# MrTornado24/IDE-3D

Measured on AMD Instinct MI355X. Metric: 512x512 RGB+seg frames/s @96 depth samples (whole job), higher is better.
Workload: dtype f32 (3x3 convs + MLPs: fp32 operands as 3 bf16 pieces, 6 products, f32 accumulate); 1 GPU; BASELINE config 2: random-init ide3d-ffhq-64-512, G.mapping + G.synthesis (64 render -> 512, 96 samples, RGB + 19-class seg) + uint8 frames, batch 4 seeds per GPU; global_batch=4, parallelism=dp1, conv_arithmetic=bf16x6, conv_arithmetic_is_library_default=True

## Files before the change

ide-3d_amd/csrc/modconv.hip:

```cpp
#include "common.h"
#include "knobs.h"
#include <stdlib.h>
#include <string.h>
#include <type_traits>

namespace ide3d {

typedef float f32x16 __attribute__((ext_vector_type(16)));

#ifdef IDE3D_MC_TRACE
__device__ unsigned long long g_mc_dbg[256];
#define IDE3D_MC_TS(k) { const unsigned long long now_ = __builtin_readcyclecounter(); mc_acc[k] += now_ - mc_last; mc_last = now_; }
#else
#define IDE3D_MC_TS(k)
#endif

enum { MODE_CONV3 = 0, MODE_CONV1 = 1, MODE_TCONV3 = 2, MODE_TCONV3A = 3, MODE_CONV3S2 = 4 };

template <int MODE> struct ModeCfg;
template <> struct ModeCfg<MODE_CONV3>  { static constexpr int KC = 4, WTAPS = 9, MAXT = 9; };
template <> struct ModeCfg<MODE_CONV1>  { static constexpr int KC = 16, WTAPS = 1, MAXT = 1; };
template <> struct ModeCfg<MODE_CONV3S2> { static constexpr int KC = 4, WTAPS = 9, MAXT = 9; };
template <> struct ModeCfg<MODE_TCONV3> { static constexpr int KC = 4, WTAPS = 9, MAXT = 4; };
template <> struct ModeCfg<MODE_TCONV3A> { static constexpr int KC = 4, WTAPS = 9, MAXT = 9; };

template <int MODE, int BIG, int TI, int PH, int PW>
struct McCfg {
    static constexpr int NWV = 4, NT = 64 * NWV;
    static constexpr int BN = TI * PH * PW;
    static_assert(BN == 64 || BN == 128 || BN == 256, "pixel tile must hold 64, 128 or 256 pixels");
    static constexpr int NCLS = (MODE == MODE_TCONV3A) ? 4 : 1;
    using MC = ModeCfg<MODE>;
    static constexpr int KC = MC::KC, WTAPS = MC::WTAPS, MAXT = MC::MAXT;
    static constexpr int WM = BIG ? 2 : 1, WN = NWV / WM;
    static constexpr int MTW = (BIG == 1) ? 2 : 1;
    static constexpr int NTW = (BN / 32) / WN;
    static constexpr int BM = WM * MTW * 32;
    static constexpr int STRIDE = (MODE == MODE_CONV3S2) ? 2 : 1;
    static constexpr int HALO = (MODE == MODE_CONV1 || MODE == MODE_CONV3S2) ? 0 : 1;
    static constexpr int HP = (MODE == MODE_CONV3S2) ? 2 * PH + 1 : PH + 2 * HALO;
    static constexpr int HW = (MODE == MODE_CONV3S2) ? 2 * PW + 1 : PW + 2 * HALO;
    static constexpr int XW = (MODE == MODE_CONV1) ? PW : (MODE == MODE_CONV3S2) ? ((HW + 3) & ~3) : ((PW == 16) ? 48 : HW + 2);
    static constexpr int XS = HP * XW;
    static constexpr int XI = KC * XS;
    static constexpr int LDS_W = MAXT * KC * BM;
    static constexpr int LDS_X = TI * XI;
    static constexpr int NW4 = (LDS_W / 4 + NT - 1) / NT;
    static constexpr int VW = (MODE == MODE_CONV1 && PH == 1 && PW % 4 == 0) ? 4 : 1;
    static constexpr int NXE = (TI * KC * HP * HW / VW + NT - 1) / NT;
};

template <int N>
__device__ __forceinline__ int sel(const int (&a)[N], int t) {
    int v = a[0];
#pragma unroll
    for (int i = 1; i < N; ++i) v = (t == i) ? a[i] : v;
    return v;
}

__host__ __device__ inline int mc_bm(int cout) { return cout > 96 ? 128 : (cout > 32 ? 64 : 32); }
__host__ __device__ inline int mc_kc(int k) { return k == 3 ? 4 : 16; }

__global__ void __launch_bounds__(256)
modconv_pack_kernel(const float* __restrict__ w, int64_t w_batch_stride, int nbatch, int cout, int cin, int taps, int bm, int kc,
                    int mblocks, int cchunks, float* __restrict__ out) {
    const int64_t total = (int64_t)nbatch * mblocks * cchunks * taps * kc * bm;
    const int64_t stride = (int64_t)gridDim.x * blockDim.x;
    for (int64_t i = (int64_t)blockIdx.x * blockDim.x + threadIdx.x; i < total; i += stride) {
        int64_t r = i;
        const int co_l = (int)(r % bm); r /= bm;
        const int cil = (int)(r % kc); r /= kc;
        const int tap = (int)(r % taps); r /= taps;
        const int cc = (int)(r % cchunks); r /= cchunks;
        const int mb = (int)(r % mblocks); r /= mblocks;
        const int nb = (int)r;
        const int co = mb * bm + co_l, ci = cc * kc + cil;
        out[i] = (co < cout && ci < cin) ? w[nb * w_batch_stride + ((int64_t)co * cin + ci) * taps + tap] : 0.f;
    }
}

struct ConvGeom {
    int tiles_x[4], tiles_y[4];
    int tile_base[5];
    int img_groups;
    int mblocks, cchunks, split_k, chunks_per_split;
    int oh, ow;
};

template <int OFF_BYTES>
__device__ __forceinline__ float lds_read_async(unsigned addr) {
    float v;
    asm volatile("ds_read_b32 %0, %1 offset:%2" : "=v"(v) : "v"(addr), "n"(OFF_BYTES));
    return v;
}
template <int PENDING>
__device__ __forceinline__ void lds_wait(float& first) { asm volatile("s_waitcnt lgkmcnt(%1)" : "+v"(first) : "n"(PENDING)); }
__device__ __forceinline__ void lds_pin(float& v) { asm volatile("" : "+v"(v)); }
__device__ __forceinline__ unsigned lds_addr(const float* p) { return (unsigned)(size_t)p; }

template <class F, int... Is>
__device__ __forceinline__ void static_for_impl(F&& f, std::integer_sequence<int, Is...>) { (f(std::integral_constant<int, Is>{}), ...); }
template <int N, class F>
__device__ __forceinline__ void static_for(F&& f) { static_for_impl(f, std::make_integer_sequence<int, N>{}); }

template <int MODE, int XW>
__host__ __device__ constexpr int tap_patch_offset(int t) {
    return (MODE == MODE_CONV1) ? 0
         : (MODE == MODE_TCONV3A) ? ((t / 3 == 2) ? 0 : 1) * XW + ((t % 3 == 2) ? 0 : 1)
         : (t / 3) * XW + (t % 3);
}
template <int MODE>
__host__ __device__ constexpr int tap_class(int t) { return (MODE == MODE_TCONV3A) ? ((t / 3) & 1) * 2 + ((t % 3) & 1) : 0; }

__device__ __forceinline__ void amax_acc(float& m, float v) { m = fmaxf(m, fabsf(v)); }
__device__ __forceinline__ void amax_commit(float* y_amax, int n, float v, bool) {
    if (v > 0.f) amax_raise(y_amax, n, v);
}

template <int MODE, int TI, int PH, int PW, int NWV, int NCLS, int MTW, int NTW, int BM, int SCRATCH, int ROWPAR = -1>
__device__ __forceinline__ void modconv_finish(const ide3d_modconv_params& p, float* __restrict__ partial, const ConvGeom& g,
                                               f32x16 (&acc)[NCLS][MTW][NTW], float* s_w, int mb, int n0, int y0, int x0, int split, int cls,
                                               int wm, int wn, int lp, const float* __restrict__ row_unscale = nullptr, float x_unscale = 1.f,
                                               int team_tid = -1, float* amax_scratch = nullptr) {
    constexpr int NT = 64 * NWV;
    const int tid = team_tid >= 0 ? team_tid : (int)threadIdx.x, lane = tid & 63, wid = tid >> 6, half = lane >> 5;
    const int cpy = cls >> 1, cpx = cls & 1;
    const bool raw = (g.split_k > 1);
    float* const s_dm = s_w;
    float* const s_bi = s_w + TI * BM;
    for (int e = tid; e < TI * BM; e += NT) {
        const int rl = e % BM, co = mb * BM + rl, n = min(n0 + e / BM, p.n - 1);
        float d = (!raw && p.dcoefs && co < p.cout) ? p.dcoefs[(int64_t)n * p.cout + co] : 1.f;
        if (row_unscale) d *= row_unscale[co] * x_unscale;
        s_dm[e] = d;
        if (e < BM) s_bi[e] = (!raw && p.bias && co < p.cout) ? p.bias[co] : 0.f;
    }
    __syncthreads();
    float* const dst = raw ? partial + (int64_t)split * p.n * p.cout * g.oh * g.ow : p.y;
    const int64_t pitch = (!raw && p.y_pitch > 0) ? p.y_pitch : g.ow;
    const float e_alpha = (!raw && p.act == 3) ? p.alpha : 1.f, e_gain = raw ? 1.f : p.gain;
    const float e_clamp = (!raw && p.clamp >= 0.f) ? p.clamp : __builtin_inff();
    const float e_nstr = (!raw && p.noise) ? p.noise_strength : 0.f;
    auto finish = [&](float v, float d, float nz, float bb) {
        v *= d; v += nz; v += bb;
        v = (v > 0.f) ? v : v * e_alpha;
        v *= e_gain;
        return fminf(fmaxf(v, -e_clamp), e_clamp);
    };
    const bool want_amax = !raw && p.y_amax != nullptr;
    float amax_tile = 0.f;
    constexpr int QX = (MODE == MODE_TCONV3A) ? 2 : 1, QY = NCLS / QX;
    static_assert(ROWPAR < 0 || (MODE == MODE_TCONV3A && NCLS == 2), "one row parity = two column classes");
    constexpr int TW = 32 * QX, TP = TW + 8;
    constexpr int AVAIL = SCRATCH - (TI + 1) * BM;
    constexpr int RR = (MODE == MODE_TCONV3 || PW % 4 != 0) ? 0 : (AVAIL >= NWV * 32 * TP) ? 32 : (AVAIL >= NWV * 16 * TP) ? 16 : (AVAIL >= NWV * 8 * TP) ? 8 : 0;
    if constexpr (RR > 0) {
        typedef float f32x4u __attribute__((ext_vector_type(4), aligned(4)));
        float* const T = s_w + (TI + 1) * BM + wid * (RR * TP);
#pragma unroll
        for (int qy = 0; qy < QY; ++qy)
#pragma unroll
// ... 958 lines not shown
        const char* src = uniform_ptr(xbase + (int64_t)t * 128);
#pragma unroll
        for (int c = 0; c < NCH; ++c)
#pragma unroll
            for (int e = 0; e < 8; ++e) {
                xr[B][c][e] = *reinterpret_cast<const float*>(src + (c * 16 + e) * plane + x_lane);
            }
    };
    typedef float f32x4a __attribute__((ext_vector_type(4)));
    const float* const bi = s_bi + 4 * half;
    f32x16 acc[MT];
    auto compute = [&](auto buf_tag) {
        constexpr int B = decltype(buf_tag)::value;
#pragma unroll
        for (int m = 0; m < MT; ++m)
#pragma unroll
            for (int g = 0; g < 4; ++g) {
                const f32x4a b4 = *reinterpret_cast<const f32x4a*>(bi + m * 32 + 8 * g);
#pragma unroll
                for (int k = 0; k < 4; ++k) acc[m][4 * g + k] = b4[k];
            }
#pragma unroll
        for (int c = 0; c < NCH; ++c) {
            u32x4 bfrag[PARTS];
            {
                unsigned pk[4][PARTS];
#pragma unroll
                for (int e = 0; e < 4; ++e) split_pair<PARTS>(xr[B][c][2 * e], xr[B][c][2 * e + 1], pk[e]);
#pragma unroll
                for (int q = 0; q < PARTS; ++q) bfrag[q] = u32x4{pk[0][q], pk[1][q], pk[2][q], pk[3][q]};
            }
            const u32x4* sa = s_a + c * K::A_UNITS + half * K::ROWS + l32;
            constexpr int MG = (MT % 2 == 0) ? 2 : 1;
#pragma unroll
            for (int m0 = 0; m0 < MT; m0 += MG) {
                u32x4 af[MG][PARTS];
#pragma unroll
                for (int g = 0; g < MG; ++g)
#pragma unroll
                    for (int q = 0; q < PARTS; ++q) af[g][q] = sa[q * 2 * K::ROWS + (m0 + g) * 32];
                constexpr int NQA = PARTS;
#pragma unroll
                for (int qa = 0; qa < NQA; ++qa)
#pragma unroll
                    for (int qb = 0; qa + qb < NQA; ++qb)
#pragma unroll
                        for (int g = 0; g < MG; ++g)
                            acc[m0 + g] = __builtin_amdgcn_mfma_f32_32x32x16_bf16(__builtin_bit_cast(bf16x8, af[g][qa]), __builtin_bit_cast(bf16x8, bfrag[qb]), acc[m0 + g], 0, 0, 0);
            }
        }
    };
    const bool all_rows = (p.cout == K::ROWS), unit_gain = (e_gain == 1.f), want_amax = (p.y_amax != nullptr);
    auto finish = [&](int t) {
        char* dst = uniform_ptr(ybase + (int64_t)t * 128);
        auto rows = [&](auto all_tag, auto gain_tag) {
            constexpr bool ALL = decltype(all_tag)::value, UNIT = decltype(gain_tag)::value;
#pragma unroll
            for (int m = 0; m < MT; ++m)
#pragma unroll
                for (int r = 0; r < 16; ++r) {
                    const int row_u = m * 32 + 8 * (r >> 2) + (r & 3);
                    if (ALL || row_u + 4 * half < p.cout) {
                        float v = acc[m][r];
                        if (!UNIT) v *= e_gain;
                        v = __builtin_amdgcn_fmed3f(v, -e_clamp, e_clamp);
                        *reinterpret_cast<float*>(dst + row_u * plane + y_lane) = v;
                        if (want_amax) amax_acc(amax, v);
                    }
                }
        };
        if (all_rows) { if (unit_gain) rows(std::true_type{}, std::true_type{}); else rows(std::true_type{}, std::false_type{}); }
        else          { if (unit_gain) rows(std::false_type{}, std::true_type{}); else rows(std::false_type{}, std::false_type{}); }
    };
    using B0 = std::integral_constant<int, 0>; using B1 = std::integral_constant<int, NBUF - 1>;
    if (wave0 < tiles32) fetch(wave0, B0{});
    asm volatile("s_waitcnt vmcnt(0)" ::: "memory");
    __syncthreads();
    if constexpr (NBUF == 1) {
        for (int t = wave0; t < tiles32; t += nwaves) {
            compute(B0{});
            if (t + nwaves < tiles32) fetch(t + nwaves, B0{});
            finish(t);
        }
    } else {
        for (int t = wave0; t < tiles32; t += 2 * nwaves) {
            if (t + nwaves < tiles32) fetch(t + nwaves, B1{});
            compute(B0{});
            finish(t);
            if (t + nwaves < tiles32) {
                if (t + 2 * nwaves < tiles32) fetch(t + 2 * nwaves, B0{});
                compute(B1{});
                finish(t + nwaves);
            }
        }
    }
    __syncthreads();
    if (p.y_amax != nullptr) amax_raise_block(p.y_amax, n0, amax, reinterpret_cast<float*>(s_a));
}


constexpr int HS_RB = 4, HS_THREADS = 1024;
template <int PX, int HS_UN>
__global__ void __launch_bounds__(HS_THREADS)
head_small_kernel(ide3d_modconv_params p, int hw) {
    constexpr int KS = HS_THREADS / PX;
    __shared__ float s_red[KS][HS_RB][PX];
    __shared__ float s_am[HS_THREADS / 64];
    const int px_l = threadIdx.x % PX;
    const int ks = __builtin_amdgcn_readfirstlane((int)(threadIdx.x / PX));
    const int row0 = blockIdx.x * HS_RB, n = blockIdx.z;
    const int px_c = min((int)blockIdx.y * PX + px_l, hw - 1);
    const int cq = (p.cin + KS - 1) / KS, c0 = ks * cq, c1 = min(c0 + cq, p.cin);
    const float* __restrict__ xl = p.x + (int64_t)n * p.cin * hw + px_c;
    const float* __restrict__ wr[HS_RB];
#pragma unroll
    for (int r = 0; r < HS_RB; ++r) wr[r] = p.w + (int64_t)n * p.w_batch_stride + (int64_t)min(row0 + r, p.cout - 1) * p.cin;
    float acc[HS_RB] = {0.f, 0.f, 0.f, 0.f};
    int c = c0;
    for (; c + HS_UN <= c1; c += HS_UN) {
        float xv[HS_UN];
#pragma unroll
        for (int e = 0; e < HS_UN; ++e) xv[e] = xl[(int64_t)(c + e) * hw];
#pragma unroll
        for (int r = 0; r < HS_RB; ++r)
#pragma unroll
            for (int e = 0; e < HS_UN; ++e) acc[r] = fmaf(xv[e], wr[r][c + e], acc[r]);
    }
    for (; c < c1; ++c) {
        const float xv = xl[(int64_t)c * hw];
#pragma unroll
        for (int r = 0; r < HS_RB; ++r) acc[r] = fmaf(xv, wr[r][c], acc[r]);
    }
#pragma unroll
    for (int r = 0; r < HS_RB; ++r) s_red[ks][r][px_l] = acc[r];
    __syncthreads();
    float amax = 0.f;
    if (threadIdx.x < HS_RB * PX) {
        const int r = threadIdx.x / PX, row = row0 + r, px = (int)blockIdx.y * PX + px_l;
        float v = s_red[0][r][px_l];
#pragma unroll
        for (int q = 1; q < KS; ++q) v += s_red[q][r][px_l];
        if (row < p.cout && px < hw) {
            if (p.bias) v += p.bias[row];
            v *= p.gain;
            if (p.clamp >= 0.f) v = fminf(fmaxf(v, -p.clamp), p.clamp);
            p.y[((int64_t)n * p.cout + row) * hw + px] = v;
            amax_acc(amax, v);
        }
    }
    if (p.y_amax != nullptr) amax_raise_block(p.y_amax, n, amax, s_am);
}


constexpr int STRIP_CO = 8, STRIP_WAVES = 16;
__global__ void __launch_bounds__(256)
tconv_strip_pack_kernel(const float* __restrict__ w, int cout, int cin, int cout_pad, float* __restrict__ ws) {
    const int64_t total = (int64_t)cin * 6 * cout_pad;
    for (int64_t i = (int64_t)blockIdx.x * 256 + threadIdx.x; i < total; i += (int64_t)gridDim.x * 256) {
        const int co = (int)(i % cout_pad); const int64_t r = i / cout_pad;
        const int t = (int)(r % 6), ci = (int)(r / 6);
        const int tap = t < 3 ? 6 + t : (t - 3) * 3 + 2;
        ws[i] = co < cout ? w[((int64_t)co * cin + ci) * 9 + tap] : 0.f;
    }
}
__global__ void __launch_bounds__(256)
tconv_strip_gather_kernel(const float* __restrict__ x, int rows, int h, int w_, float* __restrict__ xs) {
    const int len = w_ + h;
    for (int64_t i = (int64_t)blockIdx.x * 256 + threadIdx.x; i < (int64_t)rows * len; i += (int64_t)gridDim.x * 256) {
        const int64_t r = i / len; const int e = (int)(i - r * len);
        xs[i] = e < w_ ? x[r * h * w_ + (int64_t)(h - 1) * w_ + e] : x[r * h * w_ + (int64_t)(e - w_) * w_ + (w_ - 1)];
    }
}
__global__ void __launch_bounds__(64 * STRIP_WAVES, 4)
tconv_strip_kernel(ide3d_modconv_params p, const float* __restrict__ ws, const float* __restrict__ xs, int cout_pad, int oh, int ow, int64_t pitch,
                   int nb_re, int nb_ro, int nb_ce) {
    __shared__ float s_red[STRIP_WAVES][STRIP_CO][64];
    __shared__ float s_am[STRIP_WAVES];
    const int h = p.h, w_ = p.w_;
    const int lane = threadIdx.x & 63, q = __builtin_amdgcn_readfirstlane((int)(threadIdx.x >> 6));
    int b = (int)blockIdx.x, kind = 0;
    if (b >= nb_re) { b -= nb_re; kind = 1; if (b >= nb_ro) { b -= nb_ro; kind = 2; if (b >= nb_ce) { b -= nb_ce; kind = 3; } } }
    const bool is_row = kind < 2, odd = kind & 1;
    const int a = b * 64 + lane;
    const int t = 2 * a + (odd ? 1 : 0);
    const bool live = t < (is_row ? ow : oh - 1);
    const int co0 = (int)blockIdx.y * STRIP_CO, n = (int)blockIdx.z;
    const int len = is_row ? w_ : h;
    const bool ok_a = live && a < len, ok_b = live && !odd && a >= 1;
    const int64_t xs_pitch = (int64_t)w_ + h;
    const float* __restrict__ xn = xs + (int64_t)n * p.cin * xs_pitch;
    const int64_t off_a = (is_row ? 0 : w_) + min(a, len - 1), off_b = (is_row ? 0 : w_) + min(max(a - 1, 0), len - 1);
    const float* __restrict__ wt = ws + (is_row ? 0 : 3) * (int64_t)cout_pad + co0;
    constexpr int STRIP_CH = 8 * STRIP_WAVES, PER_WAVE = STRIP_CH / STRIP_WAVES, WPC = 3 * STRIP_CO;
    static_assert(PER_WAVE * WPC == 3 * 64, "three weight loads per lane and chunk");
    __shared__ __attribute__((aligned(16))) float s_wt[STRIP_WAVES][PER_WAVE * WPC];
    float acc[STRIP_CO];
#pragma unroll
    for (int j = 0; j < STRIP_CO; ++j) acc[j] = 0.f;
    for (int c0 = 0; c0 < p.cin; c0 += STRIP_CH) {
        float xa[PER_WAVE], xb[PER_WAVE], scv[PER_WAVE], wreg[3];
#pragma unroll
        for (int k = 0; k < PER_WAVE; ++k) {
            const int ci = min(c0 + q + k * STRIP_WAVES, p.cin - 1);
            xa[k] = xn[(int64_t)ci * xs_pitch + off_a];
            xb[k] = odd ? 0.f : xn[(int64_t)ci * xs_pitch + off_b];
            scv[k] = p.styles ? p.styles[(int64_t)n * p.cin + ci] : 1.f;
        }
#pragma unroll
        for (int r = 0; r < 3; ++r) {
            const int e = lane + 64 * r, k = e / WPC, rem = e - k * WPC, tp = rem / STRIP_CO, jj = rem - tp * STRIP_CO;
            const int ci = c0 + q + k * STRIP_WAVES;
            wreg[r] = (ci < p.cin) ? wt[((int64_t)ci * 6 + tp) * cout_pad + jj] : 0.f;
        }
        __builtin_amdgcn_wave_barrier();
#pragma unroll
        for (int r = 0; r < 3; ++r) s_wt[q][lane + 64 * r] = wreg[r];
        __builtin_amdgcn_fence(__ATOMIC_RELEASE, "wavefront");
        __builtin_amdgcn_wave_barrier();
        __builtin_amdgcn_fence(__ATOMIC_ACQUIRE, "wavefront");
#pragma unroll
        for (int k = 0; k < PER_WAVE; ++k) {
            const float va = ok_a ? xa[k] * scv[k] : 0.f;
            const float4* wv = reinterpret_cast<const float4*>(&s_wt[q][k * WPC]);
            if (odd) {
                const float4 b0 = wv[2], b1 = wv[3];
                const float w1[STRIP_CO] = {b0.x, b0.y, b0.z, b0.w, b1.x, b1.y, b1.z, b1.w};
#pragma unroll
                for (int j = 0; j < STRIP_CO; ++j) acc[j] = fmaf(va, w1[j], acc[j]);
            } else {
                const float vb = ok_b ? xb[k] * scv[k] : 0.f;
                const float4 a0 = wv[0], a1 = wv[1], c0v = wv[4], c1v = wv[5];
                const float w0[STRIP_CO] = {a0.x, a0.y, a0.z, a0.w, a1.x, a1.y, a1.z, a1.w};
                const float w2[STRIP_CO] = {c0v.x, c0v.y, c0v.z, c0v.w, c1v.x, c1v.y, c1v.z, c1v.w};
#pragma unroll
                for (int j = 0; j < STRIP_CO; ++j) { acc[j] = fmaf(va, w0[j], acc[j]); acc[j] = fmaf(vb, w2[j], acc[j]); }
            }
        }
    }
#pragma unroll
    for (int j = 0; j < STRIP_CO; ++j) s_red[q][j][lane] = acc[j];
    __syncthreads();
    float am = 0.f;
    {
        static_assert(STRIP_CO <= STRIP_WAVES, "wave q < STRIP_CO finishes output channel co0 + q");
        float v = 0.f;
        const int qc = min(q, STRIP_CO - 1);
#pragma unroll
        for (int k = 0; k < STRIP_WAVES; ++k) v += s_red[k][qc][lane];
        const int co = co0 + q;
        if (live && q < STRIP_CO && co < p.cout) {
            v *= p.dcoefs ? p.dcoefs[(int64_t)n * p.cout + co] : 1.f;
            const int oy = is_row ? oh - 1 : t, ox = is_row ? t : ow - 1;
            p.y[((int64_t)n * p.cout + co) * ((int64_t)oh * pitch) + (int64_t)oy * pitch + ox] = v;
            amax_acc(am, v);
        }
    }
    if (p.y_amax) amax_raise_block(p.y_amax, n, am, s_am);
}

struct BlockId { int mb, tile, grp, split; };
__device__ __forceinline__ BlockId decode_block(const ConvGeom& g) {
    int bid = xcd_remap(blockIdx.x, gridDim.x);
    BlockId b;
    b.mb = bid % g.mblocks; bid /= g.mblocks;
    b.tile = bid % g.tile_base[4]; bid /= g.tile_base[4];
    b.grp = bid % g.img_groups; bid /= g.img_groups;
    b.split = bid;
    return b;
}

template <int MODE, int BIG, int TI, int PH, int PW>
__global__ void __launch_bounds__(256, (McCfg<MODE, BIG, TI, PH, PW>::NCLS * McCfg<MODE, BIG, TI, PH, PW>::MTW * McCfg<MODE, BIG, TI, PH, PW>::NTW > 8) ? 1
                                       : (TI * PH * PW <= 128 && MODE != MODE_CONV3S2) ? 3 : 2)
modconv_kernel(ide3d_modconv_params p, const float* __restrict__ wp, float* __restrict__ partial, ConvGeom g) {
    using K = McCfg<MODE, BIG, TI, PH, PW>;
    __shared__ __attribute__((aligned(16))) float s_w[2 * K::LDS_W];
    __shared__ __attribute__((aligned(16))) float s_x[2 * K::LDS_X];
    const BlockId b = decode_block(g);
    int cls = 0;
    if (MODE == MODE_TCONV3) { cls = (b.tile >= g.tile_base[1]) + (b.tile >= g.tile_base[2]) + (b.tile >= g.tile_base[3]); }
    modconv_tile<MODE, BIG, TI, PH, PW>(p, wp, partial, g, s_w, s_x, b.mb, b.tile - g.tile_base[cls], b.grp, b.split, cls, g.tiles_x[cls]);
}


#ifdef IDE3D_SP_SHARED_SIMD
constexpr bool kSpExclusive = false;
#else
constexpr bool kSpExclusive = true;
#endif
template <int MODE, int BIG, int PH, int PARTS, int WBUF, int NWV>
constexpr int sp_waves_per_simd() {
    using K = SpCfg<MODE, BIG, PH, PARTS, WBUF, NWV>;
    return (NWV == 8) ? 2 : (!kSpExclusive && K::LDS_BYTES <= 80 * 1024 && (WBUF == 1 || K::NCLS * K::MTW * K::NTW <= 8)) ? 2 : 1;
}
template <int MODE, int BIG, int PH, int PARTS, int WBUF = 2, int NWV = 4, int F16 = 0>
__global__ void __launch_bounds__(64 * NWV, (sp_waves_per_simd<MODE, BIG, PH, PARTS, WBUF, NWV>()))
modconv_split_kernel(ide3d_modconv_params p, const u32x4* __restrict__ wp, float* __restrict__ partial, ConvGeom g, const float* __restrict__ row_unscale) {
    using K = SpCfg<MODE, BIG, PH, PARTS, WBUF, NWV>;
    if constexpr (kSpExclusive) { if constexpr (NWV == 8) asm volatile("" ::: "v255"); else asm volatile("" ::: "v255", "a255"); }
    __shared__ __attribute__((aligned(16))) unsigned char sp_smem[K::LDS_BYTES];
    const BlockId b = decode_block(g);
    modconv_split_tile<MODE, BIG, PH, PARTS, WBUF, NWV, F16>(p, wp, partial, g, sp_smem, b.mb, b.tile, b.grp, b.split, g.tiles_x[0], row_unscale);
}

template <int BIG, int PH, int HEAD_MT>
__global__ void __launch_bounds__(512, 2)
modconv_split_heads_kernel(ide3d_modconv_params p, const u32x4* __restrict__ wp, ConvGeom g, HeadEpi he) {
    using K = SpCfg<MODE_CONV3, BIG, PH, 3, 2, 8>;
    if constexpr (kSpExclusive) asm volatile("" ::: "v255");
    __shared__ __attribute__((aligned(16))) unsigned char sp_smem[K::LDS_BYTES];
    const BlockId b = decode_block(g);
    modconv_split_tile<MODE_CONV3, BIG, PH, 3, 2, 8, 0, 1, -1, HEAD_MT>(p, wp, nullptr, g, sp_smem, b.mb, b.tile, b.grp, b.split, g.tiles_x[0], nullptr, nullptr, &he);
}

template <int BIG, int PH, int PARTS, int F16 = 0>
__global__ void __launch_bounds__(512, 2)
modconv_split_pair_kernel(ide3d_modconv_params p, const u32x4* __restrict__ wp, float* __restrict__ partial, ConvGeom g, const float* __restrict__ row_unscale) {
    using K = SpCfg<MODE_TCONV3A, BIG, PH, PARTS, 2, 8, 1>;
    if constexpr (kSpExclusive) asm volatile("" ::: "v255");
    __shared__ __attribute__((aligned(16))) unsigned char sp_smem[K::LDS_BYTES];
    const int half_grid = (int)(gridDim.x >> 1);
    const int par = __builtin_amdgcn_readfirstlane((int)blockIdx.x >= half_grid ? 1 : 0);
    int bid = xcd_remap((int)blockIdx.x - par * half_grid, half_grid);
    BlockId b;
    b.mb = bid % g.mblocks; bid /= g.mblocks;
    b.tile = bid % g.tile_base[4]; bid /= g.tile_base[4];
    b.grp = bid % g.img_groups; bid /= g.img_groups;
    b.split = bid;
    if (par == 0) modconv_split_tile<MODE_TCONV3A, BIG, PH, PARTS, 2, 8, F16, 1, 0>(p, wp, partial, g, sp_smem, b.mb, b.tile, b.grp, b.split, g.tiles_x[0], row_unscale);
    else          modconv_split_tile<MODE_TCONV3A, BIG, PH, PARTS, 2, 8, F16, 1, 1>(p, wp, partial, g, sp_smem, b.mb, b.tile, b.grp, b.split, g.tiles_x[0], row_unscale);
}

template <int MODE, int BIG, int PH, int PARTS, int WBUF, int F16>
__global__ void __launch_bounds__(512, 2)
modconv_split_teams_kernel(ide3d_modconv_params p, const u32x4* __restrict__ wp, float* __restrict__ partial, ConvGeom g, const float* __restrict__ row_unscale) {
    using K = SpCfg<MODE, BIG, PH, PARTS, WBUF, 4>;
    static_assert(2 * K::LDS_BYTES <= 160 * 1024, "both teams' LDS must fit");
    asm volatile("" ::: "v255");
    __shared__ __attribute__((aligned(16))) unsigned char sp_smem[2 * K::LDS_BYTES];
    const int team = (int)(threadIdx.x >> 8);
    int bid = xcd_remap(blockIdx.x, gridDim.x);
    const int mpairs = g.mblocks >> 1;
    BlockId b;
    b.mb = 2 * (bid % mpairs) + team; bid /= mpairs;
    b.tile = bid % g.tile_base[4]; bid /= g.tile_base[4];
    b.grp = bid % g.img_groups; bid /= g.img_groups;
    b.split = bid;
    modconv_split_tile<MODE, BIG, PH, PARTS, WBUF, 4, F16, 2>(p, wp, partial, g, sp_smem + team * K::LDS_BYTES, b.mb, b.tile, b.grp, b.split, g.tiles_x[0], row_unscale,
                                                              reinterpret_cast<float*>(sp_smem));
}

__global__ void __launch_bounds__(256)
modconv_epilogue_kernel(ide3d_modconv_params p, const float* __restrict__ partial, int split_k, int oh, int ow) {
    const int64_t per = (int64_t)p.n * p.cout * oh * ow;
    const int64_t stride = (int64_t)gridDim.x * blockDim.x;
    int am_n = -1; float am = 0.f;
    __shared__ unsigned s_am[64];
    const bool am_lds = p.y_amax && p.n <= 64;
    if (p.y_amax) { if (threadIdx.x < 64) s_am[threadIdx.x] = 0u; __syncthreads(); }
    const int hw = oh * ow;
    if (p.y_pitch <= 0 && (hw & 3) == 0) {
        typedef float f32x4v __attribute__((ext_vector_type(4)));
        const int64_t per4 = per >> 2;
        for (int64_t q = (int64_t)blockIdx.x * blockDim.x + threadIdx.x; q < per4; q += stride) {
            const int64_t i = q << 2;
            f32x4v v = {0.f, 0.f, 0.f, 0.f};
            int s = 0;
            for (; s + 4 <= split_k; s += 4) {
                f32x4v t[4];
#pragma unroll
                for (int k = 0; k < 4; ++k) t[k] = *reinterpret_cast<const f32x4v*>(partial + (int64_t)(s + k) * per + i);
#pragma unroll
                for (int k = 0; k < 4; ++k) v += t[k];
            }
            for (; s < split_k; ++s) v += *reinterpret_cast<const f32x4v*>(partial + (int64_t)s * per + i);
            const int pix = (int)(i % hw);
            const int co = (int)((i / hw) % p.cout);
            const int n = (int)(i / ((int64_t)hw * p.cout));
            const float d = p.dcoefs ? p.dcoefs[(int64_t)n * p.cout + co] : 1.f, bb = p.bias ? p.bias[co] : 0.f;
#pragma unroll
            for (int e = 0; e < 4; ++e) {
                float x = v[e];
                if (p.dcoefs) x *= d;
                if (p.noise) x += p.noise[pix + e] * p.noise_strength;
                if (p.bias) x += bb;
                if (p.act == 3) x = (x > 0.f) ? x : x * p.alpha;
                x *= p.gain;
                if (p.clamp >= 0.f) x = fminf(fmaxf(x, -p.clamp), p.clamp);
                v[e] = x;
            }
            *reinterpret_cast<f32x4v*>(p.y + i) = v;
            if (p.y_amax) {
                if (n != am_n) { if (am_n >= 0) { if (am_lds) amax_lds_flush(s_am, am_n, am); else amax_commit(p.y_amax, am_n, am, false); } am_n = n; am = 0.f; }
                amax_acc(am, v[0]); amax_acc(am, v[1]); amax_acc(am, v[2]); amax_acc(am, v[3]);
            }
        }
    } else
    for (int64_t i = (int64_t)blockIdx.x * blockDim.x + threadIdx.x; i < per; i += stride) {
        float v = 0.f;
        int s = 0;
        for (; s + 8 <= split_k; s += 8) {
            float t[8];
#pragma unroll
            for (int k = 0; k < 8; ++k) t[k] = partial[(int64_t)(s + k) * per + i];
#pragma unroll
            for (int k = 0; k < 8; ++k) v += t[k];
        }
        if (s + 4 <= split_k) {
// ... 268 lines not shown
}

static bool head_split_applies(const ide3d_modconv_params& p, int arith) {
    return arith != 1 && p.k == 1 && p.mode == 0 && p.w_batch_stride > 0 && !p.styles && !p.dcoefs && !p.noise && p.act == 1 &&
           (p.cout <= 32 || (p.cout > 160 && p.cout <= 192)) && p.cin >= 32 &&
           (int64_t)p.n * ide3d::cdiv64((int64_t)p.h * p.w_, 32 * ide3d::head_waves(p.cout <= 32 ? 1 : 6)) >= ide3d::kNumCU;
}

static bool head_small_applies(const ide3d_modconv_params& p) {
    return p.k == 1 && p.mode == 0 && p.w_batch_stride > 0 && !p.styles && !p.dcoefs && !p.noise && p.act == 1 && (int64_t)p.h * p.w_ <= 256 &&
           p.y_pitch == 0 && p.n <= 65535;
}
static bool head_resident_applies(const ide3d_modconv_params& p) {
    const int mt = p.cout <= 32 ? 1 : 6, cchunks = ide3d::cdiv(p.cin, 16);
    const int hw = p.h * p.w_, wgs_img = ide3d::kNumCU / p.n, tiles32 = hw / 32;
    return ide3d::kSpExclusive && p.cin % 16 == 0 && hw % 32 == 0 && wgs_img >= 1 && p.y_pitch == 0 &&
           ((mt == 1 && (cchunks == 4 || cchunks == 8)) || (mt == 6 && cchunks == 8)) && tiles32 >= 2 * wgs_img * 8;
}

static int check_modconv(const ide3d_modconv_params& p) {
    using namespace ide3d;
    IDE3D_CHECK_ARG(p.n > 0 && p.cin > 0 && p.cout > 0 && p.h > 0 && p.w_ > 0, "modconv2d: bad shape");
    IDE3D_CHECK_ARG(p.k == 1 || p.k == 3, "modconv2d: kernel size must be 1 or 3 (got %d)", p.k);
    IDE3D_CHECK_ARG(p.mode == 0 || ((p.mode == 1 || p.mode == 2) && p.k == 3),
                    "modconv2d: mode must be 0 (conv), 1 (3x3 stride-2 conv, no padding) or 2 (3x3 transposed, stride 2)");
    IDE3D_CHECK_ARG(p.mode != 1 || (p.h >= 3 && p.w_ >= 3), "modconv2d: stride-2 convolution needs an input of at least 3x3");
    IDE3D_CHECK_ARG((int64_t)p.n * p.cin * p.h * p.w_ < 0x7fffffffLL, "modconv2d: input too large for 32-bit indexing");
    return IDE3D_OK;
}

extern "C" int64_t ide3d_modconv_workspace_bytes(int32_t n, int32_t cin, int32_t cout, int32_t h, int32_t w, int32_t k, int32_t mode,
                                                 int32_t per_image_weights) {
    using namespace ide3d;
    ide3d_modconv_params p{};
    p.n = n; p.cin = cin; p.cout = cout; p.h = h; p.w_ = w; p.k = k; p.mode = mode; p.w_batch_stride = per_image_weights ? 1 : 0;
    if (check_modconv(p) != IDE3D_OK) return -1;
    p.x = nullptr;
    int64_t packed = 0, part = 0;
    static const float dummy = 0.f;
    for (int epi = 0; epi < 2; ++epi) {
        ide3d_modconv_params q0 = p;
        q0.act = 1; q0.gain = 1.f; q0.clamp = -1.f;
        if (epi == 1) { q0.noise = &dummy; q0.bias = &dummy; q0.noise_strength = 1.f; q0.act = 3; q0.alpha = 0.2f; q0.gain = 1.41421356f; }
        for (int arith : {1, 3, 6, 16}) {
            ConvPlan pl; plan_conv(q0, pl, arith);
            ConvPlan pf; plan_conv(flatten_pointwise(q0), pf, arith);
            for (const ConvPlan* q : {&pl, &pf}) {
                if (q->packed_floats + q->aux_floats > packed) packed = q->packed_floats + q->aux_floats;
                if (q->partial_floats > part) part = q->partial_floats;
            }
        }
    }
    int64_t bytes = (packed + part) * (int64_t)sizeof(float);
    if (per_image_weights && k == 1) {
        const int64_t hb = head_packed_units(n, cdiv(cin, 16), 3, cout <= 32 ? 1 : 6) * 16;
        if (hb > bytes) bytes = hb;
    }
    return bytes;
}

static void pack_split_weights(const ide3d_modconv_params& p, const ide3d::ConvPlan& pl, float* wp, hipStream_t st) {
    using namespace ide3d;
    const int64_t items = (int64_t)pl.mblocks * pl.cchunks * 9 * 2 * pl.bm;
    if (pl.f16) {
        float* const rs = wp + pl.packed_floats;
        const int rows = pl.mblocks * pl.bm;
        hipLaunchKernelGGL(modconv_row_scale_kernel, dim3(cdiv(rows, 4)), dim3(256), 0, st, p.w, p.cout, p.cin * 9, rows, rs, rs + rows);
        hipLaunchKernelGGL((modconv_pack_split_kernel<2, 1>), dim3(stream_grid(items, 256)), dim3(256), 0, st, p.w, p.cout, p.cin, pl.bm, pl.mblocks, pl.cchunks, reinterpret_cast<u32x4*>(wp), rs);
    }
    else if (pl.parts == 2) hipLaunchKernelGGL(modconv_pack_split_kernel<2>, dim3(stream_grid(items, 256)), dim3(256), 0, st, p.w, p.cout, p.cin, pl.bm, pl.mblocks, pl.cchunks, reinterpret_cast<u32x4*>(wp), nullptr);
    else               hipLaunchKernelGGL(modconv_pack_split_kernel<3>, dim3(stream_grid(items, 256)), dim3(256), 0, st, p.w, p.cout, p.cin, pl.bm, pl.mblocks, pl.cchunks, reinterpret_cast<u32x4*>(wp), nullptr);
}

extern "C" int ide3d_modconv2d(const ide3d_modconv_params* pp, void* stream) {
    using namespace ide3d;
    IDE3D_CHECK_ARG(pp != nullptr, "modconv2d: null params");
    const ide3d_modconv_params p = flatten_pointwise(*pp);
    IDE3D_CHECK_ARG(p.x && p.w && p.y && p.workspace, "modconv2d: null tensor / workspace pointer");
    int rc = check_modconv(p);
    if (rc) return rc;
    IDE3D_CHECK_ARG(p.act == 1 || p.act == 3, "modconv2d: act must be linear (1) or lrelu (3)");
    IDE3D_CHECK_ARG(p.y_pitch == 0 || (p.mode == 2 && p.y_pitch >= 2 * p.w_ + 1), "modconv2d: y_pitch is the row pitch of a transposed convolution's output (>= 2 w + 1), or 0");
    hipStream_t st_head = (hipStream_t)stream;
    {
        const int64_t hw = (int64_t)p.h * p.w_;
        if (head_small_applies(p)) {
            if (hw <= 64) hipLaunchKernelGGL((head_small_kernel<64, 32>), dim3(cdiv(p.cout, HS_RB), 1, p.n), dim3(HS_THREADS), 0, st_head, p, (int)hw);
            else          hipLaunchKernelGGL((head_small_kernel<256, 8>), dim3(cdiv(p.cout, HS_RB), cdiv((int)hw, 256), p.n), dim3(HS_THREADS), 0, st_head, p, (int)hw);
            IDE3D_CHECK_LAUNCH("modconv2d (small-map heads)");
            return IDE3D_OK;
        }
    }
    if (head_split_applies(p, resolve_arith(p.arith))) {
        const int parts = resolve_arith(p.arith) == 3 ? 2 : 3, mt = p.cout <= 32 ? 1 : 6, cchunks = cdiv(p.cin, 16);
        IDE3D_CHECK_ARG(p.workspace_bytes >= head_packed_units(p.n, cchunks, parts, mt) * 16, "modconv2d: workspace too small for the packed head weights");
        u32x4* wu = reinterpret_cast<u32x4*>(p.workspace);
        const int64_t items = (int64_t)p.n * cchunks * 2 * mt * 32;
        const int tiles = cdiv(p.h * p.w_, 32 * head_waves(mt));
        const int hw_h = p.h * p.w_, wgs_img = kNumCU / p.n, tiles32 = hw_h / 32;
        const bool resident = head_resident_applies(p);
#define IDE3D_HEAD_RES(P, M, C) IDE3D_EXCL_LAUNCH((head_resident_kernel<P, M, C>), dim3(p.n * wgs_img), 512, 0, st_head, p, wu, wgs_img, tiles32)
#define IDE3D_HEAD(P, M) do { \
            hipLaunchKernelGGL(head_pack_split_kernel<P>, dim3(stream_grid(items, 256)), dim3(256), 0, st_head, p.w, p.w_batch_stride, p.n, p.cout, p.cin, M * 32, cchunks, wu); \
            if (resident) { if (M == 6) IDE3D_HEAD_RES(P, 6, 8); else if (cchunks == 4) IDE3D_HEAD_RES(P, 1, 4); else IDE3D_HEAD_RES(P, 1, 8); } \
            else IDE3D_EXCL_LAUNCH((head_split_kernel<P, M>), dim3(p.n * tiles), 64 * head_waves(M), 0, st_head, p, wu, cchunks, tiles); } while (0)
        if (parts == 2) { if (mt == 1) IDE3D_HEAD(2, 1); else IDE3D_HEAD(2, 6); }
        else            { if (mt == 1) IDE3D_HEAD(3, 1); else IDE3D_HEAD(3, 6); }
#undef IDE3D_HEAD
#undef IDE3D_HEAD_RES
        IDE3D_CHECK_LAUNCH("modconv2d (split-bf16 heads)");
        return IDE3D_OK;
    }
    int arith_eff = resolve_arith(p.arith);
    if (arith_eff == 16 && !p.x_amax) arith_eff = 6;
    ConvPlan pl; plan_conv(p, pl, arith_eff);
    IDE3D_CHECK_ARG(p.workspace_bytes >= (pl.packed_floats + pl.aux_floats + pl.partial_floats) * (int64_t)sizeof(float),
                    "modconv2d: workspace too small (need %lld bytes)", (long long)((pl.packed_floats + pl.aux_floats + pl.partial_floats) * sizeof(float)));
    hipStream_t st = (hipStream_t)stream;
    float* wp = p.workspace;
    float* partial = p.workspace + pl.packed_floats + pl.aux_floats;
    if (pl.parts) {
        if (!p.weights_packed) pack_split_weights(p, pl, wp, st);
#define IDE3D_SP_DISPATCH(M) \
        do { if (pl.big == 1) { if (pl.f16) launch_split<M, 1, 2, 1>(p, pl, wp, partial, st); else if (pl.parts == 2) launch_split<M, 1, 2>(p, pl, wp, partial, st); else launch_split<M, 1, 3>(p, pl, wp, partial, st); } \
             else             { if (pl.f16) launch_split<M, 2, 2, 1>(p, pl, wp, partial, st); else if (pl.parts == 2) launch_split<M, 2, 2>(p, pl, wp, partial, st); else launch_split<M, 2, 3>(p, pl, wp, partial, st); } } while (0)
        if (pl.mode == MODE_CONV3) IDE3D_SP_DISPATCH(MODE_CONV3); else IDE3D_SP_DISPATCH(MODE_TCONV3A);
#undef IDE3D_SP_DISPATCH
    } else {
    if (!p.weights_packed) {
        hipLaunchKernelGGL(modconv_pack_kernel, dim3(stream_grid(pl.packed_floats, 256)), dim3(256), 0, st,
                           p.w, p.w_batch_stride, p.w_batch_stride ? p.n : 1, p.cout, p.cin, pl.taps, pl.bm, pl.kc, pl.mblocks, pl.cchunks, wp);
    }
#define IDE3D_MC_DISPATCH(M) \
    do { if (pl.big == 1) launch_tiles<M, 1>(p, pl, wp, partial, st); else if (pl.big == 2) launch_tiles<M, 2>(p, pl, wp, partial, st); \
         else launch_tiles<M, 0>(p, pl, wp, partial, st); } while (0)
    if (pl.mode == MODE_CONV3)       IDE3D_MC_DISPATCH(MODE_CONV3);
    else if (pl.mode == MODE_CONV1)  IDE3D_MC_DISPATCH(MODE_CONV1);
    else if (pl.mode == MODE_CONV3S2) IDE3D_MC_DISPATCH(MODE_CONV3S2);
    else if (pl.mode == MODE_TCONV3A) IDE3D_MC_DISPATCH(MODE_TCONV3A);
    else                             IDE3D_MC_DISPATCH(MODE_TCONV3);
#undef IDE3D_MC_DISPATCH
    }
    if (pl.g.split_k > 1) {
        const int64_t per = (int64_t)p.n * p.cout * pl.oh * pl.ow;
        hipLaunchKernelGGL(modconv_epilogue_kernel, dim3(stream_grid((p.y_pitch <= 0 && ((pl.oh * pl.ow) & 3) == 0) ? per / 4 : per, 256)), dim3(256), 0, st, p, partial, pl.g.split_k, pl.oh, pl.ow);
    }
    if (pl.mode == MODE_TCONV3A && !p.weights_packed) {
        hipLaunchKernelGGL(tconv_strip_pack_kernel, dim3(stream_grid(pl.strip_floats, 256)), dim3(256), 0, st, p.w, p.cout, p.cin, cdiv(p.cout, STRIP_CO) * STRIP_CO,
                           wp + pl.packed_floats + pl.strip_off);
    }
    if (pl.strip) {
        const int cout_pad = cdiv(p.cout, STRIP_CO) * STRIP_CO;
        float* const wstrip = wp + pl.packed_floats + pl.strip_off;
        const int nb_re = cdiv(p.w_ + 1, 64), nb_ro = cdiv(p.w_, 64), nb_ce = cdiv(p.h, 64), nb_co = cdiv(p.h, 64);
        float* const xs = wstrip + pl.strip_floats;
        hipLaunchKernelGGL(tconv_strip_gather_kernel, dim3(stream_grid((int64_t)p.n * p.cin * (p.h + p.w_), 256)), dim3(256), 0, st, p.x, p.n * p.cin, p.h, p.w_, xs);
        hipLaunchKernelGGL(tconv_strip_kernel, dim3(nb_re + nb_ro + nb_ce + nb_co, cout_pad / STRIP_CO, p.n), dim3(64 * STRIP_WAVES), 0, st, p, wstrip, xs, cout_pad,
                           pl.oh, pl.ow, (int64_t)(p.y_pitch > 0 ? p.y_pitch : pl.ow), nb_re, nb_ro, nb_ce);
    }
    IDE3D_CHECK_LAUNCH("modconv2d");
    return IDE3D_OK;
}

extern "C" int ide3d_modconv2d_heads(const ide3d_modconv_params* pp, const ide3d_modconv_head_epilogue* hp, void* stream) {
    using namespace ide3d;
    IDE3D_CHECK_ARG(pp != nullptr && hp != nullptr, "modconv2d_heads: null params");
    const ide3d_modconv_params& p = *pp;
    const ide3d_modconv_head_epilogue& h = *hp;
    IDE3D_CHECK_ARG(p.x && p.w && p.workspace && (p.y || h.no_activation_output) && h.w && h.y && h.workspace, "modconv2d_heads: null tensor / workspace pointer");
    int rc = check_modconv(p);
    if (rc) return rc;
    IDE3D_CHECK_ARG(p.act == 1 || p.act == 3, "modconv2d_heads: act must be linear (1) or lrelu (3)");
    IDE3D_CHECK_ARG(h.rows > 0, "modconv2d_heads: bad head rows");
    auto no_kernel = [](const char* why) { set_error("modconv2d_heads: %s", why); return IDE3D_ENOKERNEL; };
    if (knob_live("IDE3D_MODCONV_NO_HEAD_FUSION")) return no_kernel("IDE3D_MODCONV_NO_HEAD_FUSION is set");
    if (p.k != 3 || p.mode != 0 || p.w_batch_stride != 0 || p.y_amax || p.y_pitch != 0) return no_kernel("not a shared-weight 3x3 layer without side outputs");
    int arith = resolve_arith(p.arith);
    if (arith == 16 && !p.x_amax) arith = 6;
    if (arith != 6) return no_kernel("the fused form exists for bf16x6 only");
    ConvPlan pl; plan_conv(p, pl, arith);
    if (pl.parts != 3 || pl.f16 || pl.mode != MODE_CONV3 || pl.pair || pl.g.split_k != 1 || pl.g.mblocks != 1 || pl.bm != p.cout || kTiles[pl.tile].images != 1)
        return no_kernel("the layer's plan does not hold all channels of a tile in one workgroup");
    const bool tile16 = pl.big == 1 && p.cout == 128 && pl.tile == T16x16 && sp_form(pl).waves == 8;
    const bool tile32 = pl.big == 2 && p.cout == 64 && pl.tile == T32x16;
    const int ph = tile32 ? 32 : 16;
    if (!(tile16 || tile32) || p.h % ph != 0 || p.w_ % 16 != 0) return no_kernel("no fused instance for this tile");
    ide3d_modconv_params q{};
    q.x = p.y; q.w = h.w; q.bias = h.bias; q.y = h.y;
    q.n = p.n; q.cin = p.cout; q.cout = h.rows; q.h = p.h; q.w_ = p.w_; q.k = 1; q.mode = 0;
    q.act = 1; q.alpha = 0.f; q.gain = 1.f; q.clamp = h.clamp; q.w_batch_stride = (int64_t)h.rows * p.cout; q.arith = p.arith;
    const int mt = h.rows <= 32 ? 1 : 6, hcc = p.cout / 16;
    if (head_small_applies(q) || !head_split_applies(q, resolve_arith(q.arith)) || resolve_arith(q.arith) == 3 || (mt == 6 && !tile16))
        return no_kernel("the heads do not take the split-bf16 path");
    IDE3D_CHECK_ARG(p.workspace_bytes >= (pl.packed_floats + pl.aux_floats) * (int64_t)sizeof(float), "modconv2d_heads: workspace too small");
    IDE3D_CHECK_ARG(h.workspace_bytes >= head_packed_units(p.n, hcc, 3, mt) * 16, "modconv2d_heads: head workspace too small");
    hipStream_t st = (hipStream_t)stream;
    if (!p.weights_packed) pack_split_weights(p, pl, p.workspace, st);
    u32x4* const hw_packed = reinterpret_cast<u32x4*>(h.workspace);
    const int64_t items = (int64_t)p.n * hcc * 2 * mt * 32;
    hipLaunchKernelGGL(head_pack_split_kernel<3>, dim3(stream_grid(items, 256)), dim3(256), 0, st, h.w, q.w_batch_stride, p.n, h.rows, p.cout, mt * 32, hcc, hw_packed);
    HeadEpi e;
    e.w = hw_packed; e.bias = h.bias; e.y = h.y; e.rows = h.rows; e.clamp = h.clamp; e.store_x = !h.no_activation_output;
    e.bias_first = head_resident_applies(q) ? 1 : 0;
    const ConvGeom& g = pl.g;
    const unsigned nblocks = (unsigned)((int64_t)g.mblocks * g.tile_base[4] * g.img_groups * g.split_k);
    const u32x4* wu = reinterpret_cast<const u32x4*>(p.workspace);
    if (tile32) IDE3D_EXCL_LAUNCH((modconv_split_heads_kernel<2, 32, 1>), dim3(nblocks), 512, 0, st, p, wu, g, e);
    else if (mt == 1) IDE3D_EXCL_LAUNCH((modconv_split_heads_kernel<1, 16, 1>), dim3(nblocks), 512, 0, st, p, wu, g, e);
    else IDE3D_EXCL_LAUNCH((modconv_split_heads_kernel<1, 16, 6>), dim3(nblocks), 512, 0, st, p, wu, g, e);
    IDE3D_CHECK_LAUNCH("modconv2d_heads");
    return IDE3D_OK;
}

extern "C" int ide3d_modconv_plan(const ide3d_modconv_params* pp, ide3d_modconv_plan_info* out) {
    using namespace ide3d;
    IDE3D_CHECK_ARG(pp != nullptr && out != nullptr, "modconv_plan: null argument");
    const ide3d_modconv_params p = flatten_pointwise(*pp);
    int rc = check_modconv(p);
    if (rc) return rc;
    *out = ide3d_modconv_plan_info{};
    const int arith = resolve_arith(p.arith);
    if (head_small_applies(p)) {
        const int hw = p.h * p.w_;
        out->kind = IDE3D_PLAN_HEAD_SMALL; out->tile_h = 1; out->tile_w = hw <= 64 ? 64 : 256; out->rows = HS_RB; out->waves = HS_THREADS / 64; out->split_k = 1;
        out->workgroups = (int64_t)cdiv(p.cout, HS_RB) * (hw <= 64 ? 1 : cdiv(hw, 256)) * p.n;
        return IDE3D_OK;
    }
    if (head_split_applies(p, arith)) {
        const int mt = p.cout <= 32 ? 1 : 6;
        out->rows = mt * 32; out->parts = arith == 3 ? 2 : 3; out->split_k = 1; out->tile_h = 1;
        if (head_resident_applies(p)) { out->kind = IDE3D_PLAN_HEAD_RESIDENT; out->tile_w = 32; out->waves = 8; out->workgroups = (int64_t)p.n * (kNumCU / p.n); }
        else { out->kind = IDE3D_PLAN_HEAD_SPLIT; out->waves = head_waves(mt); out->tile_w = 32 * out->waves; out->workgroups = (int64_t)p.n * cdiv(p.h * p.w_, out->tile_w); }
        return IDE3D_OK;
    }
    int arith_eff = arith;
    if (arith_eff == 16 && !p.x_amax) arith_eff = 6;
    ConvPlan pl; plan_conv(p, pl, arith_eff);
    const int64_t blocks = (int64_t)pl.g.mblocks * pl.g.tile_base[4] * pl.g.img_groups * pl.g.split_k * (pl.pair ? 2 : 1);
    out->tile_h = kTiles[pl.tile].rows; out->tile_w = kTiles[pl.tile].cols; out->images_per_tile = kTiles[pl.tile].images;
    out->rows = pl.bm; out->parts = pl.parts; out->f16 = pl.f16; out->split_k = pl.g.split_k; out->strip = pl.strip;
    out->transposed_all_class = (pl.mode == MODE_TCONV3A);
    if (pl.parts) {
        const SpForm f = sp_form(pl);
        out->kind = f.teams ? IDE3D_PLAN_SPLIT_TEAMS : IDE3D_PLAN_SPLIT; out->waves = f.teams ? 8 : f.waves; out->workgroups = f.teams ? blocks / 2 : blocks;
    } else {
        out->kind = IDE3D_PLAN_FP32; out->waves = 4; out->workgroups = blocks;
    }
    return IDE3D_OK;
}

extern "C" int ide3d_set_conv_arithmetic(int32_t arith) {
    IDE3D_CHECK_ARG(arith == 0 || arith == 1 || arith == 3 || arith == 6 || arith == 16,
                    "set_conv_arithmetic: 0 (environment default), 1 (fp32), 3 (bf16x3), 6 (bf16x6) or 16 (f16x3)");
    ide3d::g_conv_arith = arith;
    return IDE3D_OK;
}
extern "C" int32_t ide3d_get_conv_arithmetic(void) { return ide3d::conv_arith_default(); }

#ifdef IDE3D_MC_TRACE
extern "C" int ide3d_debug_mc(unsigned long long* host) {
    return (int)hipMemcpyFromSymbol(host, HIP_SYMBOL(ide3d::g_mc_dbg), sizeof(unsigned long long) * 256);
}
#endif

namespace ide3d {
const char* modconv_build_flags() {
    return ""
#ifdef IDE3D_SP_SHARED_SIMD
        "!IDE3D_SP_SHARED_SIMD "
#endif
#ifdef IDE3D_MC_TRACE
        "IDE3D_MC_TRACE "
#endif
        ;
}
}
```

Measured before the change: 952.5 frames/s.

## Rewrite transposed-conv edge strip kernel on f32 MFMA and drop gather pass

Reimplements the edge-strip kernel of the transposed 3x3 conv with __builtin_amdgcn_mfma_f32_16x16x4f32 instead of per-lane scalar FMAs. Each block now covers 16 positions and computes both output parities together, for 64 output channels per block. Inputs are read straight from the activation tensor with a strided column walk, so the separate gather kernel and its scratch traffic are skipped by default. The cost is a two-pass shared-memory reduction across 8 waves, strided uncoalesced column loads, and a new output-channel mapping that could hide indexing errors.

```diff
diff --git a/ide-3d_amd/csrc/modconv.hip b/ide-3d_amd/csrc/modconv.hip
--- a/ide-3d_amd/csrc/modconv.hip
+++ b/ide-3d_amd/csrc/modconv.hip
@@ -7,6 +7,7 @@
 namespace ide3d {
 
 typedef float f32x16 __attribute__((ext_vector_type(16)));
+typedef float f32x4 __attribute__((ext_vector_type(4)));
 
 #ifdef IDE3D_MC_TRACE
 __device__ unsigned long long g_mc_dbg[256];
@@ -1271,7 +1272,9 @@
 }
 
 
-constexpr int STRIP_CO = 8, STRIP_WAVES = 16;
+constexpr int STRIP_CO = 8;
+constexpr int STRIP_WAVES = 8, STRIP_POS = 16;
+constexpr int STRIP_MT = 4;
 __global__ void __launch_bounds__(256)
 tconv_strip_pack_kernel(const float* __restrict__ w, int cout, int cin, int cout_pad, float* __restrict__ ws) {
     const int64_t total = (int64_t)cin * 6 * cout_pad;
@@ -1290,89 +1293,86 @@
         xs[i] = e < w_ ? x[r * h * w_ + (int64_t)(h - 1) * w_ + e] : x[r * h * w_ + (int64_t)(e - w_) * w_ + (w_ - 1)];
     }
 }
-__global__ void __launch_bounds__(64 * STRIP_WAVES, 4)
-tconv_strip_kernel(ide3d_modconv_params p, const float* __restrict__ ws, const float* __restrict__ xs, int cout_pad, int oh, int ow, int64_t pitch,
-                   int nb_re, int nb_ro, int nb_ce) {
-    __shared__ float s_red[STRIP_WAVES][STRIP_CO][64];
+static bool strip_gathers(const ide3d_modconv_params&) { return false; }
+struct StripSrc { const float* xsrc; int64_t img, ch, row, col, col_step; };
+template <int MT>
+__global__ void __launch_bounds__(64 * STRIP_WAVES)
+tconv_strip_kernel(ide3d_modconv_params p, const float* __restrict__ ws, StripSrc src, int cout_pad, int oh, int ow, int64_t pitch, int nb_row) {
+    __shared__ float s_red[STRIP_WAVES][MT * 4][64];
     __shared__ float s_am[STRIP_WAVES];
-    const int h = p.h, w_ = p.w_;
     const int lane = threadIdx.x & 63, q = __builtin_amdgcn_readfirstlane((int)(threadIdx.x >> 6));
-    int b = (int)blockIdx.x, kind = 0;
-    if (b >= nb_re) { b -= nb_re; kind = 1; if (b >= nb_ro) { b -= nb_ro; kind = 2; if (b >= nb_ce) { b -= nb_ce; kind = 3; } } }
-    const bool is_row = kind < 2, odd = kind & 1;
-    const int a = b * 64 + lane;
-    const int t = 2 * a + (odd ? 1 : 0);
-    const bool live = t < (is_row ? ow : oh - 1);
-    const int co0 = (int)blockIdx.y * STRIP_CO, n = (int)blockIdx.z;
-    const int len = is_row ? w_ : h;
-    const bool ok_a = live && a < len, ok_b = live && !odd && a >= 1;
-    const int64_t xs_pitch = (int64_t)w_ + h;
-    const float* __restrict__ xn = xs + (int64_t)n * p.cin * xs_pitch;
-    const int64_t off_a = (is_row ? 0 : w_) + min(a, len - 1), off_b = (is_row ? 0 : w_) + min(max(a - 1, 0), len - 1);
-    const float* __restrict__ wt = ws + (is_row ? 0 : 3) * (int64_t)cout_pad + co0;
-    constexpr int STRIP_CH = 8 * STRIP_WAVES, PER_WAVE = STRIP_CH / STRIP_WAVES, WPC = 3 * STRIP_CO;
-    static_assert(PER_WAVE * WPC == 3 * 64, "three weight loads per lane and chunk");
-    __shared__ __attribute__((aligned(16))) float s_wt[STRIP_WAVES][PER_WAVE * WPC];
-    float acc[STRIP_CO];
-#pragma unroll
-    for (int j = 0; j < STRIP_CO; ++j) acc[j] = 0.f;
-    for (int c0 = 0; c0 < p.cin; c0 += STRIP_CH) {
-        float xa[PER_WAVE], xb[PER_WAVE], scv[PER_WAVE], wreg[3];
-#pragma unroll
-        for (int k = 0; k < PER_WAVE; ++k) {
-            const int ci = min(c0 + q + k * STRIP_WAVES, p.cin - 1);
-            xa[k] = xn[(int64_t)ci * xs_pitch + off_a];
-            xb[k] = odd ? 0.f : xn[(int64_t)ci * xs_pitch + off_b];
-            scv[k] = p.styles ? p.styles[(int64_t)n * p.cin + ci] : 1.f;
-        }
-#pragma unroll
-        for (int r = 0; r < 3; ++r) {
-            const int e = lane + 64 * r, k = e / WPC, rem = e - k * WPC, tp = rem / STRIP_CO, jj = rem - tp * STRIP_CO;
-            const int ci = c0 + q + k * STRIP_WAVES;
-            wreg[r] = (ci < p.cin) ? wt[((int64_t)ci * 6 + tp) * cout_pad + jj] : 0.f;
-        }
-        __builtin_amdgcn_wave_barrier();
-#pragma unroll
-        for (int r = 0; r < 3; ++r) s_wt[q][lane + 64 * r] = wreg[r];
-        __builtin_amdgcn_fence(__ATOMIC_RELEASE, "wavefront");
-        __builtin_amdgcn_wave_barrier();
-        __builtin_amdgcn_fence(__ATOMIC_ACQUIRE, "wavefront");
-#pragma unroll
-        for (int k = 0; k < PER_WAVE; ++k) {
-            const float va = ok_a ? xa[k] * scv[k] : 0.f;
-            const float4* wv = reinterpret_cast<const float4*>(&s_wt[q][k * WPC]);
-            if (odd) {
-                const float4 b0 = wv[2], b1 = wv[3];
-                const float w1[STRIP_CO] = {b0.x, b0.y, b0.z, b0.w, b1.x, b1.y, b1.z, b1.w};
-#pragma unroll
-                for (int j = 0; j < STRIP_CO; ++j) acc[j] = fmaf(va, w1[j], acc[j]);
-            } else {
-                const float vb = ok_b ? xb[k] * scv[k] : 0.f;
-                const float4 a0 = wv[0], a1 = wv[1], c0v = wv[4], c1v = wv[5];
-                const float w0[STRIP_CO] = {a0.x, a0.y, a0.z, a0.w, a1.x, a1.y, a1.z, a1.w};
-                const float w2[STRIP_CO] = {c0v.x, c0v.y, c0v.z, c0v.w, c1v.x, c1v.y, c1v.z, c1v.w};
-#pragma unroll
-                for (int j = 0; j < STRIP_CO; ++j) { acc[j] = fmaf(va, w0[j], acc[j]); acc[j] = fmaf(vb, w2[j], acc[j]); }
-            }
-        }
-    }
-#pragma unroll
-    for (int j = 0; j < STRIP_CO; ++j) s_red[q][j][lane] = acc[j];
-    __syncthreads();
+    int b = (int)blockIdx.x;
+    const bool is_row = b < nb_row;
+    if (!is_row) b -= nb_row;
+    const int len = is_row ? p.w_ : p.h;
+    const int a0 = b * STRIP_POS, co0 = (int)blockIdx.y * (16 * MT), n = (int)blockIdx.z;
+    const int kq = lane >> 4, l16 = lane & 15, a = a0 + l16;
+    const bool ok_a = a < len, ok_b = a >= 1 && a - 1 < len;
+    const int64_t step = is_row ? 1 : src.col_step;
+    const float* __restrict__ xl = src.xsrc + (int64_t)n * src.img + (is_row ? src.row : src.col);
+    const float* __restrict__ wt = ws + (is_row ? 0 : 3) * (int64_t)cout_pad;
+    const float* __restrict__ st = p.styles ? p.styles + (int64_t)n * p.cin : nullptr;
+    f32x4 even[MT], odd[MT];
+#pragma unroll
+    for (int mt = 0; mt < MT; ++mt) { even[mt] = f32x4{0.f, 0.f, 0.f, 0.f}; odd[mt] = f32x4{0.f, 0.f, 0.f, 0.f}; }
+    const int ksteps = cdiv(p.cin, 4);
+    constexpr int UN = 2;
+    for (int ks0 = q; ks0 < ksteps; ks0 += UN * STRIP_WAVES) {
+        float xa[UN], xb[UN], wa[UN][MT][3];
+#pragma unroll
+        for (int u = 0; u < UN; ++u) {
+            const int ci = 4 * (ks0 + u * STRIP_WAVES) + kq;
+            const bool ok_c = ci < p.cin;
+            const float* __restrict__ xc = xl + (int64_t)ci * src.ch;
+            xa[u] = (ok_c && ok_a) ? xc[(int64_t)a * step] : 0.f;
+            xb[u] = (ok_c && ok_b) ? xc[(int64_t)(a - 1) * step] : 0.f;
+            if (st) {
+                const float sc = ok_c ? st[ci] : 0.f;
+                xa[u] = (ok_c && ok_a) ? xa[u] * sc : 0.f;
+                xb[u] = (ok_c && ok_b) ? xb[u] * sc : 0.f;
+            }
+#pragma unroll
+            for (int mt = 0; mt < MT; ++mt) {
+                const int co = co0 + 16 * mt + l16;
+                const bool ok_w = ok_c && co < cout_pad;
+#pragma unroll
+                for (int tp = 0; tp < 3; ++tp) wa[u][mt][tp] = ok_w ? wt[((int64_t)ci * 6 + tp) * cout_pad + co] : 0.f;
+            }
+        }
+#pragma unroll
+        for (int u = 0; u < UN; ++u)
+#pragma unroll
+            for (int mt = 0; mt < MT; ++mt) {
+                if (co0 + 16 * mt < p.cout) {
+                    even[mt] = __builtin_amdgcn_mfma_f32_16x16x4f32(wa[u][mt][0], xa[u], even[mt], 0, 0, 0);
+                    odd[mt]  = __builtin_amdgcn_mfma_f32_16x16x4f32(wa[u][mt][1], xa[u], odd[mt], 0, 0, 0);
+                    even[mt] = __builtin_amdgcn_mfma_f32_16x16x4f32(wa[u][mt][2], xb[u], even[mt], 0, 0, 0);
+                }
+            }
+    }
     float am = 0.f;
-    {
-        static_assert(STRIP_CO <= STRIP_WAVES, "wave q < STRIP_CO finishes output channel co0 + q");
-        float v = 0.f;
-        const int qc = min(q, STRIP_CO - 1);
-#pragma unroll
-        for (int k = 0; k < STRIP_WAVES; ++k) v += s_red[k][qc][lane];
-        const int co = co0 + q;
-        if (live && q < STRIP_CO && co < p.cout) {
-            v *= p.dcoefs ? p.dcoefs[(int64_t)n * p.cout + co] : 1.f;
-            const int oy = is_row ? oh - 1 : t, ox = is_row ? t : ow - 1;
-            p.y[((int64_t)n * p.cout + co) * ((int64_t)oh * pitch) + (int64_t)oy * pitch + ox] = v;
-            amax_acc(am, v);
-        }
+#pragma unroll
+    for (int par = 0; par < 2; ++par) {
+#pragma unroll
+        for (int mt = 0; mt < MT; ++mt)
+#pragma unroll
+            for (int r = 0; r < 4; ++r) s_red[q][mt * 4 + r][lane] = par ? odd[mt][r] : even[mt][r];
+        __syncthreads();
+        for (int e = (int)threadIdx.x; e < MT * 4 * 64; e += 64 * STRIP_WAVES) {
+            const int slot = e >> 6, l = e & 63;
+            float v = s_red[0][slot][l];
+#pragma unroll
+            for (int k = 1; k < STRIP_WAVES; ++k) v += s_red[k][slot][l];
+            const int co = co0 + 16 * (slot >> 2) + 4 * (l >> 4) + (slot & 3);
+            const int t = 2 * (a0 + (l & 15)) + par;
+            if (t < (is_row ? ow : oh - 1) && co < p.cout) {
+                v *= p.dcoefs ? p.dcoefs[(int64_t)n * p.cout + co] : 1.f;
+                const int oy = is_row ? oh - 1 : t, ox = is_row ? t : ow - 1;
+                p.y[((int64_t)n * p.cout + co) * ((int64_t)oh * pitch) + (int64_t)oy * pitch + ox] = v;
+                amax_acc(am, v);
+            }
+        }
+        __syncthreads();
     }
     if (p.y_amax) amax_raise_block(p.y_amax, n, am, s_am);
 }
@@ -1947,11 +1947,15 @@
     if (pl.strip) {
         const int cout_pad = cdiv(p.cout, STRIP_CO) * STRIP_CO;
         float* const wstrip = wp + pl.packed_floats + pl.strip_off;
-        const int nb_re = cdiv(p.w_ + 1, 64), nb_ro = cdiv(p.w_, 64), nb_ce = cdiv(p.h, 64), nb_co = cdiv(p.h, 64);
-        float* const xs = wstrip + pl.strip_floats;
-        hipLaunchKernelGGL(tconv_strip_gather_kernel, dim3(stream_grid((int64_t)p.n * p.cin * (p.h + p.w_), 256)), dim3(256), 0, st, p.x, p.n * p.cin, p.h, p.w_, xs);
-        hipLaunchKernelGGL(tconv_strip_kernel, dim3(nb_re + nb_ro + nb_ce + nb_co, cout_pad / STRIP_CO, p.n), dim3(64 * STRIP_WAVES), 0, st, p, wstrip, xs, cout_pad,
-                           pl.oh, pl.ow, (int64_t)(p.y_pitch > 0 ? p.y_pitch : pl.ow), nb_re, nb_ro, nb_ce);
+        StripSrc src{p.x, (int64_t)p.cin * p.h * p.w_, (int64_t)p.h * p.w_, (int64_t)(p.h - 1) * p.w_, p.w_ - 1, p.w_};
+        if (strip_gathers(p)) {
+            float* const xs = wstrip + pl.strip_floats;
+            hipLaunchKernelGGL(tconv_strip_gather_kernel, dim3(stream_grid((int64_t)p.n * p.cin * (p.h + p.w_), 256)), dim3(256), 0, st, p.x, p.n * p.cin, p.h, p.w_, xs);
+            src = StripSrc{xs, (int64_t)p.cin * (p.h + p.w_), (int64_t)p.h + p.w_, 0, p.w_, 1};
+        }
+        const int nb_row = cdiv(p.w_ + 1, STRIP_POS), nb_col = cdiv(p.h, STRIP_POS);
+        hipLaunchKernelGGL(tconv_strip_kernel<STRIP_MT>, dim3(nb_row + nb_col, cdiv(p.cout, 16 * STRIP_MT), p.n), dim3(64 * STRIP_WAVES), 0, st, p, wstrip, src, cout_pad,
+                           pl.oh, pl.ow, (int64_t)(p.y_pitch > 0 ? p.y_pitch : pl.ow), nb_row);
     }
     IDE3D_CHECK_LAUNCH("modconv2d");
     return IDE3D_OK;
```

Result: no change. 954.0 frames/s (median of 6 runs) (+0.2%).
